# OpenNLPLab/ACR_WSSS

Measured on NVIDIA B200. Metric: train_imgs_per_sec, higher is better.
Workload: dtype bf16

## Files before the change

### acr_wsss_b200/csrc/attn_tc.cu

```cuda
#include "attn_tc.cuh"
#include <cstdlib>

using namespace acr_attn;

namespace {

struct FwdSmem {
  uint8_t q[TILE_BYTES];
  uint8_t k[2][TILE_BYTES];
  uint8_t v[2][TILE_BYTES];
  float mx[2][2][BM];
  float lsum[2][BM];
  uint64_t q_full, kv_full[2], kv_empty[2], s_full, s_free, p_full, o_full;
  uint32_t tmem_base;
};

constexpr float kRescaleThreshold = 8.f;
constexpr int FWD_THREADS = 384;
__device__ __forceinline__ void fwd_pair_sync(int quad) {
  switch (quad) {
    case 0: asm volatile("bar.sync 1, 64;" ::: "memory"); break;
    case 1: asm volatile("bar.sync 2, 64;" ::: "memory"); break;
    case 2: asm volatile("bar.sync 3, 64;" ::: "memory"); break;
    default: asm volatile("bar.sync 4, 64;" ::: "memory"); break;
  }
}
__global__ void __launch_bounds__(FWD_THREADS, 2)
attn_fwd_kernel(const __grid_constant__ CUtensorMap tmap_qkv, __nv_bfloat16* __restrict__ out, float* __restrict__ lse,
                int N, int H, float scale_log2) {
  extern __shared__ uint8_t smem_raw[];
  FwdSmem& s = *reinterpret_cast<FwdSmem*>((reinterpret_cast<uintptr_t>(smem_raw) + 1023) & ~(uintptr_t)1023);
  const int warp = threadIdx.x >> 5, lane = threadIdx.x & 31;
  const int q0 = blockIdx.x * BM, h = blockIdx.y, b = blockIdx.z;
  const int ntiles = (N + BN - 1) / BN;

  if (warp == 0 && lane == 0) {
    tc::prefetch_tmap(&tmap_qkv);
    tc::mbar_init(&s.q_full, 1);
    for (int i = 0; i < 2; ++i) { tc::mbar_init(&s.kv_full[i], 1); tc::mbar_init(&s.kv_empty[i], 1); }
    tc::mbar_init(&s.s_full, 1);
    tc::mbar_init(&s.s_free, 256);
    tc::mbar_init(&s.p_full, 256);
    tc::mbar_init(&s.o_full, 1);
    tc::fence_barrier_init();
  }
  if (warp == 2) tc::tmem_alloc<256>(&s.tmem_base);
  tc::tc_fence_before();
  __syncthreads();
  tc::tc_fence_after();
  const uint32_t tmem = s.tmem_base;
  const uint32_t tS = tmem, tP = tmem + 128, tO = tmem + 192;

  if (warp == 0) {
    tc::reg_dealloc<40>();
    if (tc::elect_one()) {
      tc::mbar_arrive_expect_tx(&s.q_full, TILE_BYTES);
      tc::tma_load_4d(s.q, &tmap_qkv, &s.q_full, 0, h, q0, b);
    }
    __syncwarp();
    for (int j = 0; j < ntiles; ++j) {
      const int st = j & 1;
      tc::mbar_wait(&s.kv_empty[st], ((j >> 1) & 1) ^ 1);
      if (tc::elect_one()) {
        tc::mbar_arrive_expect_tx(&s.kv_full[st], 2 * TILE_BYTES);
        tc::tma_load_4d(s.k[st], &tmap_qkv, &s.kv_full[st], 0, H + h, j * BN, b);
        tc::tma_load_4d(s.v[st], &tmap_qkv, &s.kv_full[st], 0, 2 * H + h, j * BN, b);
      }
      __syncwarp();
    }
  } else if (warp == 1) {
    tc::reg_dealloc<40>();
    tc::mbar_wait(&s.q_full, 0);
    const uint64_t qd = tc::smem_desc_sw128(tc::smem_u32(s.q), 16, 1024);
    auto issue_s = [&](int j) {
      const uint64_t kd = tc::smem_desc_sw128(tc::smem_u32(s.k[j & 1]), 16, 1024);
      if (tc::elect_one()) {
#pragma unroll
        for (int ks = 0; ks < HD / 16; ++ks) tc::mma_ss_off(tS, qd, ks * 2, kd, ks * 2, IDESC_S, ks > 0);
        tc::tc_commit(&s.s_full);
      }
      __syncwarp();
    };
    tc::mbar_wait(&s.kv_full[0], 0);
    tc::tc_fence_after();
    issue_s(0);
    for (int j = 0; j < ntiles; ++j) {
      const int st = j & 1;
      if (j + 1 < ntiles) {
        tc::mbar_wait(&s.kv_full[(j + 1) & 1], ((j + 1) >> 1) & 1);
        tc::mbar_wait(&s.s_free, j & 1);
        tc::tc_fence_after();
        issue_s(j + 1);
      }
      tc::mbar_wait(&s.p_full, j & 1);
      tc::tc_fence_after();
      const uint64_t vd = tc::smem_desc_sw128(tc::smem_u32(s.v[st]), 1024, 1024);
      if (tc::elect_one()) {
#pragma unroll
        for (int ks = 0; ks < BN / 16; ++ks) tc::mma_ts_off(tO, tP + ks * 8, vd, ks * 128, IDESC_PV, (j > 0) || (ks > 0));
        tc::tc_commit(&s.o_full);
        tc::tc_commit(&s.kv_empty[st]);
      }
      __syncwarp();
    }
  } else if (warp < 4) {
    tc::reg_dealloc<40>();
  } else {
    tc::reg_alloc<96>();
    const int half = (warp - 4) >> 2;
    const int quad = warp & 3;
    const int row = quad * 32 + lane;
    const uint32_t lane_off = (uint32_t)(quad * 32) << 16;
    const int cb = half * 64;
    float m = -INFINITY, l = 0.f;
    uint32_t r[32];
    const bool rows_live = q0 + quad * 32 < N;
    for (int j = 0; j < ntiles; ++j) {
      tc::mbar_wait(&s.s_full, j & 1);
      tc::tc_fence_after();
      if (!rows_live) {
        tc::tc_fence_before();
        tc::mbar_arrive(&s.s_free);
        tc::mbar_arrive(&s.p_full);
        tc::mbar_wait(&s.p_full, j & 1);
        continue;
      }
      const int ncols = min(BN, N - j * BN);
      const bool full = (ncols == BN);
      float mx = -INFINITY;
#pragma unroll
      for (int c = 0; c < 2; ++c) {
        const int c0 = cb + c * 32;
        if (c0 < ncols) {
          tc::tmem_ld32(tS + lane_off + c0, r);
          tc::tmem_ld_wait();
          if (full) {
#pragma unroll
            for (int i = 0; i < 32; ++i) mx = fmaxf(mx, __uint_as_float(r[i]));
          } else {
#pragma unroll
            for (int i = 0; i < 32; ++i) mx = fmaxf(mx, (c0 + i < ncols) ? __uint_as_float(r[i]) : -INFINITY);
          }
        }
      }
      s.mx[j & 1][half][row] = mx;
      fwd_pair_sync(quad);
      mx = fmaxf(mx, s.mx[j & 1][half ^ 1][row]);
      if (j > 0) {
        tc::mbar_wait(&s.o_full, (j - 1) & 1);
        tc::tc_fence_after();
      }
      if (j == 0) {
        m = mx;
      } else {
        const bool need = (mx - m) * scale_log2 > kRescaleThreshold;
        if (__any_sync(0xffffffffu, need)) {
          const float alpha = need ? tc::fast_exp2((m - mx) * scale_log2) : 1.f;
          if (need) { m = mx; l *= alpha; }
          tc::tmem_ld32(tO + lane_off + half * 32, r);
          tc::tmem_ld_wait();
#pragma unroll
          for (int i = 0; i < 32; ++i) r[i] = __float_as_uint(__uint_as_float(r[i]) * alpha);
          tc::tmem_st16(tO + lane_off + half * 32, r);
          tc::tmem_st16(tO + lane_off + half * 32 + 16, r + 16);
        }
      }
      const float ms = m * scale_log2;
      const uint64_t sc2 = tc::f2_pack(scale_log2, scale_log2), nms2 = tc::f2_pack(-ms, -ms);
      uint64_t rs2 = tc::f2_pack(0.f, 0.f);
#pragma unroll
      for (int c = 0; c < 2; ++c) {
        const int c0 = cb + c * 32;
        const bool any = c0 < ncols;
        if (any) {
          tc::tmem_ld32(tS + lane_off + c0, r);
          tc::tmem_ld_wait();
        }
        if (c == 1) {
          tc::tc_fence_before();
          tc::mbar_arrive(&s.s_free);
        }
        uint32_t pk[16];
        if (any) {
#pragma unroll
          for (int i = 0; i < 16; ++i) {
            float x0, x1;
            tc::f2_unpack(tc::f2_fma(tc::f2_pack(__uint_as_float(r[2 * i]), __uint_as_float(r[2 * i + 1])), sc2, nms2), x0, x1);
            float p0 = tc::fast_exp2(x0), p1 = tc::fast_exp2(x1);
            if (!full) {
              if (c0 + 2 * i >= ncols) p0 = 0.f;
              if (c0 + 2 * i + 1 >= ncols) p1 = 0.f;
            }
            rs2 = tc::f2_add(rs2, tc::f2_pack(p0, p1));
            pk[i] = tc::pack_bf16(p0, p1);
          }
        } else {
#pragma unroll
          for (int i = 0; i < 16; ++i) pk[i] = 0u;
        }
        tc::tmem_st16(tP + lane_off + half * 32 + c * 16, pk);
      }
      tc::tmem_st_wait();
      tc::tc_fence_before();
      tc::mbar_arrive(&s.p_full);
      float rs_lo, rs_hi;
      tc::f2_unpack(rs2, rs_lo, rs_hi);
      l += rs_lo + rs_hi;
    }
    if (rows_live) {
      s.lsum[half][row] = l;
      fwd_pair_sync(quad);
      l += s.lsum[half ^ 1][row];
      tc::mbar_wait(&s.o_full, (ntiles - 1) & 1);
      tc::tc_fence_after();
      tc::tmem_ld32(tO + lane_off + half * 32, r);
      tc::tmem_ld_wait();
      if (q0 + row < N) {
        const float inv = 1.f / l;
        __nv_bfloat16* dst = out + ((size_t)b * N + q0 + row) * ((size_t)H * HD) + (size_t)h * HD + half * 32;
#pragma unroll
        for (int c = 0; c < 4; ++c) {
          uint4 v;
          v.x = tc::pack_bf16(__uint_as_float(r[c * 8 + 0]) * inv, __uint_as_float(r[c * 8 + 1]) * inv);
          v.y = tc::pack_bf16(__uint_as_float(r[c * 8 + 2]) * inv, __uint_as_float(r[c * 8 + 3]) * inv);
          v.z = tc::pack_bf16(__uint_as_float(r[c * 8 + 4]) * inv, __uint_as_float(r[c * 8 + 5]) * inv);
          v.w = tc::pack_bf16(__uint_as_float(r[c * 8 + 6]) * inv, __uint_as_float(r[c * 8 + 7]) * inv);
          reinterpret_cast<uint4*>(dst)[c] = v;
        }
        if (half == 0) lse[((size_t)b * H + h) * N + q0 + row] = (m * scale_log2 + log2f(l)) * kLn2;
      }
    }
  }
  tc::tc_fence_before();
  __syncthreads();
  if (warp == 2) {
    tc::tc_fence_after();
    tc::tmem_dealloc<256>(tmem);
  }
}

constexpr int MEAN_STAGES = 3;
constexpr int MEAN_SW_SLICES = 4;
struct MeanSmem {
  uint8_t qk[MEAN_STAGES][2][TILE_BYTES];
  float lse2[MEAN_MAX_H][BM];
  float part[MEAN_SW_SLICES][MEAN_MAX_H][BM];
  uint64_t full[MEAN_STAGES], empty[MEAN_STAGES], t_full[2], t_empty[2];
  uint32_t tmem_base;
};
constexpr int STAGE_LD = 129;
static_assert(sizeof(float) * BM * STAGE_LD <= sizeof(uint8_t) * MEAN_STAGES * 2 * TILE_BYTES, "staging tile must fit");

constexpr int MEAN_SW = 16;
static_assert(MEAN_SW == 4 * MEAN_SW_SLICES, "slices of the softmax warps");
constexpr int MEAN_COLS = BN / (MEAN_SW / 4);
constexpr int MEAN_THREADS = 128 + MEAN_SW * 32;

template <int MODE>
__global__ void __launch_bounds__(MEAN_THREADS, 1)
attn_mean_kernel(const __grid_constant__ CUtensorMap tmap_qkv, const float* __restrict__ lse, float* __restrict__ mean,
                 long long mean_bs, long long mean_ld, GCode gc, float* __restrict__ p_row0, int N, int H, float scale_log2) {
  extern __shared__ uint8_t smem_raw[];
  MeanSmem& s = *reinterpret_cast<MeanSmem*>((reinterpret_cast<uintptr_t>(smem_raw) + 1023) & ~(uintptr_t)1023);
  const int warp = threadIdx.x >> 5, lane = threadIdx.x & 31;
  const int kv0 = blockIdx.x * BN, q0 = blockIdx.y * BM, b = blockIdx.z;

  if (warp == 0 && lane == 0) {
    tc::prefetch_tmap(&tmap_qkv);
    for (int i = 0; i < MEAN_STAGES; ++i) { tc::mbar_init(&s.full[i], 1); tc::mbar_init(&s.empty[i], 1); }
    for (int i = 0; i < 2; ++i) { tc::mbar_init(&s.t_full[i], 1); tc::mbar_init(&s.t_empty[i], MEAN_SW * 32); }
    tc::fence_barrier_init();
  }
  if (warp == 2) tc::tmem_alloc<256>(&s.tmem_base);
  tc::tc_fence_before();
  __syncthreads();
  tc::tc_fence_after();
  const uint32_t tmem = s.tmem_base;

  if (warp == 0) {
    for (int h = 0; h < H; ++h) {
      const int st = h % MEAN_STAGES;
      tc::mbar_wait(&s.empty[st], ((h / MEAN_STAGES) & 1) ^ 1);
      if (tc::elect_one()) {
        tc::mbar_arrive_expect_tx(&s.full[st], 2 * TILE_BYTES);
        tc::tma_load_4d(s.qk[st][0], &tmap_qkv, &s.full[st], 0, h, q0, b);
        tc::tma_load_4d(s.qk[st][1], &tmap_qkv, &s.full[st], 0, H + h, kv0, b);
      }
      __syncwarp();
    }
  } else if (warp == 1) {
    for (int h = 0; h < H; ++h) {
      const int st = h % MEAN_STAGES, ab = h & 1;
      tc::mbar_wait(&s.full[st], (h / MEAN_STAGES) & 1);
      tc::mbar_wait(&s.t_empty[ab], ((h >> 1) & 1) ^ 1);
      tc::tc_fence_after();
      const uint64_t qd = tc::smem_desc_sw128(tc::smem_u32(s.qk[st][0]), 16, 1024), kd = tc::smem_desc_sw128(tc::smem_u32(s.qk[st][1]), 16, 1024);
      if (tc::elect_one()) {
#pragma unroll
        for (int ks = 0; ks < HD / 16; ++ks) tc::mma_ss_off(tmem + ab * 128, qd, ks * 2, kd, ks * 2, IDESC_S, ks > 0);
        tc::tc_commit(&s.empty[st]);
        tc::tc_commit(&s.t_full[ab]);
      }
      __syncwarp();
    }
  } else if (warp >= 4) {
    const int we = warp - 4;
    const int row = (warp & 3) * 32 + lane;
    const int slice = we >> 2;
    const int sidx = we * 32 + lane;
    const uint32_t lane_off = (uint32_t)((warp & 3) * 32) << 16;
    const bool row_ok = (q0 + row) < N;
    const int col0 = kv0 + slice * MEAN_COLS;
    float acc[MEAN_COLS];
    const float invH = 1.f / (float)H;
    if (MODE == 0) {
#pragma unroll
      for (int i = 0; i < MEAN_COLS; ++i) acc[i] = 0.f;
    } else if (gc.ptr == nullptr) {
      const float* grow = mean + (size_t)b * mean_bs + (size_t)(q0 + row) * mean_ld + col0;
#pragma unroll
      for (int i = 0; i < MEAN_COLS; ++i) acc[i] = (row_ok && col0 + i < N) ? __ldg(grow + i) * invH : 0.f;
    } else {
      const float w2 = gcode_weight(gc, q0 + row, invH);
      const uint4* crow = reinterpret_cast<const uint4*>(gc.ptr + (size_t)b * gc.bs + (size_t)min(q0 + row, N - 1) * gc.ld + col0);
#pragma unroll
      for (int v = 0; v < MEAN_COLS / 16; ++v) {
        const uint4 t = __ldg(crow + v);
        const uint32_t w[4] = {t.x, t.y, t.z, t.w};
#pragma unroll
        for (int j = 0; j < 4; ++j)
#pragma unroll
          for (int k = 0; k < 4; ++k) {
            const int i = v * 16 + j * 4 + k;
            acc[i] = (row_ok && col0 + i < N) ? ACR_CODE_F(w[j], k) * w2 : 0.f;
          }
      }
    }
    {
      constexpr int HSTEP = MEAN_SW * 32 / BM;
      const int rr = sidx & (BM - 1);
      const bool ok = (q0 + rr) < N;
      const float* lp = lse + (size_t)b * H * N + q0 + rr;
      for (int h0 = sidx / BM; h0 < H; h0 += HSTEP * 4) {
        float v[4];
#pragma unroll
        for (int k = 0; k < 4; ++k) v[k] = (ok && h0 + HSTEP * k < H) ? __ldg(lp + (size_t)(h0 + HSTEP * k) * N) : INFINITY;
#pragma unroll
        for (int k = 0; k < 4; ++k)
          if (h0 + HSTEP * k < H) s.lse2[h0 + HSTEP * k][rr] = v[k] * kLog2e;
      }
    }
    asm volatile("bar.sync 1, %0;" ::"n"(MEAN_SW * 32) : "memory");
    const bool tail = (kv0 + BN > N);
    const bool row0_warp = (MODE == 0) && (p_row0 != nullptr) && (q0 == 0) && ((warp & 3) == 0);
    const bool live = (q0 + (warp & 3) * 32 < N) && (col0 < N);
    uint32_t r[32];
    for (int h = 0; h < H; ++h) {
      const int ab = h & 1;
      const float lse2 = s.lse2[h][row];
      tc::mbar_wait(&s.t_full[ab], (h >> 1) & 1);
      tc::tc_fence_after();
      float part = 0.f;
#pragma unroll
      for (int c = 0; c < MEAN_COLS / 32; ++c) {
        const int colbase = col0 + c * 32;
        if (!live || (tail && colbase >= N)) break;
        tc::tmem_ld32(tmem + ab * 128 + lane_off + slice * MEAN_COLS + c * 32, r);
        tc::tmem_ld_wait();
        if (!tail) {
          const uint64_t sc2 = tc::f2_pack(scale_log2, scale_log2), nl2 = tc::f2_pack(-lse2, -lse2);
          uint64_t part2 = tc::f2_pack(0.f, 0.f);
#pragma unroll
          for (int i = 0; i < 32; i += 2) {
            float x0, x1;
            tc::f2_unpack(tc::f2_fma(tc::f2_pack(__uint_as_float(r[i]), __uint_as_float(r[i + 1])), sc2, nl2), x0, x1);
            const float p0 = tc::fast_exp2(x0), p1 = tc::fast_exp2(x1);
            const uint64_t pp = tc::f2_pack(p0, p1), aa = tc::f2_pack(acc[c * 32 + i], acc[c * 32 + i + 1]);
            if (MODE == 0) {
              tc::f2_unpack(tc::f2_add(aa, pp), acc[c * 32 + i], acc[c * 32 + i + 1]);
              r[i] = __float_as_uint(p0); r[i + 1] = __float_as_uint(p1);
            } else {
              part2 = tc::f2_fma(pp, aa, part2);
            }
          }
          if (MODE == 1) { float a0, a1; tc::f2_unpack(part2, a0, a1); part += a0 + a1; }
        } else {
#pragma unroll
          for (int i = 0; i < 32; ++i) {
            float p = tc::fast_exp2(fmaf(__uint_as_float(r[i]), scale_log2, -lse2));
            if (colbase + i >= N) p = 0.f;
            if (MODE == 0) { acc[c * 32 + i] += p; r[i] = __float_as_uint(p); } else part = fmaf(p, acc[c * 32 + i], part);
          }
        }
        if (row0_warp && lane == 0) {
          float* dst0 = p_row0 + ((size_t)b * H + h) * N + colbase;
#pragma unroll
          for (int i = 0; i < 32; ++i)
            if (colbase + i < N) dst0[i] = __uint_as_float(r[i]);
        }
      }
      tc::tc_fence_before();
      tc::mbar_arrive(&s.t_empty[ab]);
      if (MODE == 1) s.part[slice][h][row] = part;
    }
    if (MODE == 1) {
      asm volatile("bar.sync 1, %0;" ::"n"(MEAN_SW * 32) : "memory");
      float* plane = p_row0 + (size_t)blockIdx.x * gridDim.z * H * N;
      for (int idx = sidx; idx < H * BM; idx += MEAN_SW * 32) {
        const int hh = idx / BM, rr = idx % BM;
        if (q0 + rr < N) {
          float v = 0.f;
#pragma unroll
          for (int sl = 0; sl < MEAN_SW_SLICES; ++sl) v += s.part[sl][hh][rr];
          plane[((size_t)b * H + hh) * N + q0 + rr] = v;
        }
      }
    }
    if (MODE == 0) {
    float* stage = reinterpret_cast<float*>(&s.qk[0][0][0]);
#pragma unroll
    for (int i = 0; i < MEAN_COLS; ++i) stage[row * STAGE_LD + slice * MEAN_COLS + i] = acc[i] * invH;
    asm volatile("bar.sync 1, %0;" ::"n"(MEAN_SW * 32) : "memory");
    float* dst = mean + (size_t)b * mean_bs;
    constexpr int RPW = BM / MEAN_SW;
#pragma unroll 1
    for (int r4 = we * RPW; r4 < we * RPW + RPW; r4 += 4) {
      if (q0 + r4 >= N) break;
      float v[4][4];
#pragma unroll
      for (int u = 0; u < 4; ++u)
#pragma unroll
        for (int cc = 0; cc < 4; ++cc) v[u][cc] = stage[(r4 + u) * STAGE_LD + cc * 32 + lane];
#pragma unroll
      for (int u = 0; u < 4; ++u) {
        if (q0 + r4 + u < N) {
#pragma unroll
          for (int cc = 0; cc < 4; ++cc) {
            const int col = cc * 32 + lane;
            if (kv0 + col < N) dst[(size_t)(q0 + r4 + u) * N + kv0 + col] = v[u][cc];
          }
        }
      }
    }
    }
  }
  tc::tc_fence_before();
  __syncthreads();
  if (warp == 2) {
    tc::tc_fence_after();
    tc::tmem_dealloc<256>(tmem);
  }
}

}

namespace acr_attn {
EncodeTiledFn get_encode_fn() {
  static EncodeTiledFn fn = nullptr;
  if (!fn) {
    void* p = nullptr;
    cudaDriverEntryPointQueryResult qres;
    if (cudaGetDriverEntryPoint("cuTensorMapEncodeTiled", &p, cudaEnableDefault, &qres) != cudaSuccess || qres != cudaDriverEntryPointSuccess)
      return nullptr;
    fn = (EncodeTiledFn)p;
  }
  return fn;
}

int make_tmap(CUtensorMap* m, const void* base, int B, int N, int SH, int D) {
  EncodeTiledFn fn = get_encode_fn();
  ACR_REQUIRE(fn != nullptr, ACR_E_NOSM100, "cuTensorMapEncodeTiled unavailable");
  cuuint64_t dims[4] = {(cuuint64_t)D, (cuuint64_t)SH, (cuuint64_t)N, (cuuint64_t)B};
  cuuint64_t strides[3] = {(cuuint64_t)D * 2, (cuuint64_t)SH * D * 2, (cuuint64_t)N * SH * D * 2};
  cuuint32_t box[4] = {(cuuint32_t)D, 1, (cuuint32_t)BM, 1};
  cuuint32_t estr[4] = {1, 1, 1, 1};
  CUresult r = fn(m, CU_TENSOR_MAP_DATA_TYPE_BFLOAT16, 4, const_cast<void*>(base), dims, strides, box, estr, CU_TENSOR_MAP_INTERLEAVE_NONE,
                  CU_TENSOR_MAP_SWIZZLE_128B, CU_TENSOR_MAP_L2_PROMOTION_L2_256B, CU_TENSOR_MAP_FLOAT_OOB_FILL_NONE);
  ACR_REQUIRE(r == CUDA_SUCCESS, ACR_E_INVAL, "cuTensorMapEncodeTiled failed (%d)", (int)r);
  return 0;
}

}

extern "C" int acr_attn_fwd_bf16(const void* qkv, int B, int N, int H, int D, float scale,
                                 void* out, float* lse, float* attn_mean, long long mean_batch_stride,
                                 float* p_row0, void* stream) {
  ACR_REQUIRE(qkv && out && lse, ACR_E_INVAL, "acr_attn_fwd_bf16: null pointer");
  ACR_REQUIRE(B > 0 && N > 0 && H > 0, ACR_E_INVAL, "acr_attn_fwd_bf16: bad shape");
  ACR_REQUIRE(D == HD, ACR_E_INVAL, "acr_attn_fwd_bf16: head dim %d unsupported (64 only)", D);
  ACR_REQUIRE(B <= 65535 && H <= MEAN_MAX_H, ACR_E_INVAL, "acr_attn_fwd_bf16: B <= 65535 and H <= %d required", MEAN_MAX_H);
  ACR_REQUIRE(((uintptr_t)qkv & 15) == 0 && ((uintptr_t)out & 15) == 0, ACR_E_ALIGN, "acr_attn_fwd_bf16: qkv/out must be 16-byte aligned");
  ACR_REQUIRE(p_row0 == nullptr || attn_mean != nullptr, ACR_E_INVAL, "acr_attn_fwd_bf16: p_row0 needs attn_mean");
  ACR_REQUIRE(acr_device_is_sm100(), ACR_E_NOSM100, "acr_attn_fwd_bf16: needs an sm_100 device");
  cudaStream_t st = (cudaStream_t)stream;
  CUtensorMap tmap;
  if (int e = make_tmap(&tmap, qkv, B, N, 3 * H, D)) return e;
  const float scale_log2 = scale * kLog2e;
  const int qt = (N + BM - 1) / BM, kt = (N + BN - 1) / BN;
  {
    const size_t smem = sizeof(FwdSmem) + 1024;
    static bool attr_set[64] = {false};
    if (int e = set_max_smem(attn_fwd_kernel, smem, attr_set)) return e;
    dim3 grid(qt, H, B);
    acr::KernelTimer kt_("attn_fwd_kernel", st);
    attn_fwd_kernel<<<grid, FWD_THREADS, smem, st>>>(tmap, (__nv_bfloat16*)out, lse, N, H, scale_log2);
    if (int e = acr::check_launch("attn_fwd_kernel")) return e;
  }
  if (attn_mean) {
    const size_t smem = sizeof(MeanSmem) + 1024;
    static bool attr_set[64] = {false};
    if (int e = set_max_smem(attn_mean_kernel<0>, smem, attr_set)) return e;
    dim3 grid(kt, qt, B);
    acr::KernelTimer kt_("attn_mean_kernel", st);
    attn_mean_kernel<0><<<grid, MEAN_THREADS, smem, st>>>(tmap, lse, attn_mean, mean_batch_stride, (long long)N, GCode{}, p_row0, N, H, scale_log2);
    if (int e = acr::check_launch("attn_mean_kernel")) return e;
  }
  return 0;
}


namespace {


__global__ void __launch_bounds__(256)
bwd_delta_kernel(const __nv_bfloat16* __restrict__ out, const __nv_bfloat16* __restrict__ d_out, const float* __restrict__ part,
                 int nparts, float* __restrict__ delta, float4* __restrict__ dq_acc, int* __restrict__ dq_bad, long long rows, int N, int H) {
  const int lane = threadIdx.x & 31;
  const long long t = ((long long)blockIdx.x * (blockDim.x >> 5) + (threadIdx.x >> 5)) * 4 + (lane >> 3);
  const bool ok = t < rows;
  float acc = 0.f;
  if (ok) {
    const uint4 a = __ldg(reinterpret_cast<const uint4*>(out + t * HD) + (lane & 7));
    const uint4 d = __ldg(reinterpret_cast<const uint4*>(d_out + t * HD) + (lane & 7));
    const __nv_bfloat162* a2 = reinterpret_cast<const __nv_bfloat162*>(&a);
    const __nv_bfloat162* d2 = reinterpret_cast<const __nv_bfloat162*>(&d);
#pragma unroll
    for (int i = 0; i < 4; ++i) {
      const float2 fa = __bfloat1622float2(a2[i]), fd = __bfloat1622float2(d2[i]);
      acc = fmaf(fa.x, fd.x, acc);
      acc = fmaf(fa.y, fd.y, acc);
    }
    const float4 z = make_float4(0.f, 0.f, 0.f, 0.f);
#pragma unroll
    for (int m = 0; m < 4; ++m) dq_acc[t * (HD / 2) + m * 8 + (lane & 7)] = z;
  }
  acc += __shfl_xor_sync(0xffffffffu, acc, 1);
  acc += __shfl_xor_sync(0xffffffffu, acc, 2);
  acc += __shfl_xor_sync(0xffffffffu, acc, 4);
  if (ok && (lane & 7) == 0) {
    const int h = (int)(t % H);
    const long long bn = t / H;
    const int n = (int)(bn % N), b = (int)(bn / N);
    const size_t idx = ((size_t)b * H + h) * N + n;
    for (int k = 0; k < nparts; ++k) acc += __ldg(part + (size_t)k * rows + idx);
    delta[idx] = acc;
    dq_bad[idx] = 0;
  }
}

__global__ void __launch_bounds__(256)
bwd_dq_convert_kernel(const long long* __restrict__ dq_acc, const int* __restrict__ dq_bad, __nv_bfloat16* __restrict__ d_qkv, int B, int N,
                      int H, float scale) {
  const long long t = (long long)blockIdx.x * blockDim.x + threadIdx.x;
  if (t >= (long long)B * H * N * (HD / 8)) return;
  const int c = (int)(t % (HD / 8));
  const long long row = t / (HD / 8);
  const int n = (int)(row % N);
  const int h = (int)((row / N) % H);
  const int b = (int)(row / ((long long)N * H));
  const longlong2* src = reinterpret_cast<const longlong2*>(dq_acc + row * HD + c * 8);
  const float sc = __ldg(dq_bad + row) ? __int_as_float(0x7fc00000) : scale * kDqUnfix;
  float x[8];
#pragma unroll
  for (int j = 0; j < 4; ++j) {
    const longlong2 q = __ldg(src + j);
    x[2 * j] = __ll2float_rn(q.x) * sc;
    x[2 * j + 1] = __ll2float_rn(q.y) * sc;
  }
  uint4 v;
  v.x = tc::pack_bf16(x[0], x[1]);
  v.y = tc::pack_bf16(x[2], x[3]);
  v.z = tc::pack_bf16(x[4], x[5]);
  v.w = tc::pack_bf16(x[6], x[7]);
  *reinterpret_cast<uint4*>(d_qkv + (((size_t)b * N + n) * 3 + 0) * ((size_t)H * HD) + (size_t)h * HD + c * 8) = v;
}

}

extern "C" size_t acr_attn_bwd_bf16_workspace(int B, int N, int H, int D) {
  if (B <= 0 || N <= 0 || H <= 0 || D <= 0) return 0;
  const size_t rows = (size_t)B * H * N, kt = (N + BN - 1) / BN;
  return acr::align_up(rows * sizeof(float), 256) + acr::align_up(rows * D * sizeof(long long), 256) + acr::align_up(kt * rows * sizeof(float), 256) +
         acr::align_up(rows * sizeof(int), 256);
}

extern "C" int acr_attn_bwd_bf16(const void* qkv, const void* out, const float* lse, const void* d_out,
                                 int B, int N, int H, int D, float scale,
                                 const float* g_mean, long long g_batch_stride, long long g_row_stride,
                                 const unsigned char* g_code, long long code_batch_stride, long long code_row_stride,
                                 float w_cls, float w_aff, const float* g_scale,
                                 void* d_qkv, float* g_row0, void* workspace, size_t workspace_bytes, void* stream) {
  ACR_REQUIRE(qkv && out && lse && d_out && d_qkv && workspace, ACR_E_INVAL, "acr_attn_bwd_bf16: null pointer");
  ACR_REQUIRE(B > 0 && N > 0 && H > 0, ACR_E_INVAL, "acr_attn_bwd_bf16: bad shape");
  ACR_REQUIRE(D == HD, ACR_E_INVAL, "acr_attn_bwd_bf16: head dim %d unsupported (64 only)", D);
  ACR_REQUIRE(B <= 65535 && H <= MEAN_MAX_H, ACR_E_INVAL, "acr_attn_bwd_bf16: B <= 65535 and H <= %d required", MEAN_MAX_H);
  ACR_REQUIRE(g_mean == nullptr || g_row_stride >= N, ACR_E_INVAL, "acr_attn_bwd_bf16: g_row_stride < N");
  ACR_REQUIRE(g_mean == nullptr || g_code == nullptr, ACR_E_INVAL, "acr_attn_bwd_bf16: give g_mean OR g_code");
  ACR_REQUIRE(g_code == nullptr || ((code_row_stride % 128) == 0 && code_row_stride >= (long long)((N + 127) / 128) * 128 &&
                                    (code_batch_stride % 16) == 0 && ((uintptr_t)g_code & 15) == 0),
              ACR_E_ALIGN, "acr_attn_bwd_bf16: g_code rows must be 128-byte padded and 16-byte aligned");
  const GCode gc{g_code, code_batch_stride, code_row_stride, w_cls, w_aff, g_scale};
  ACR_REQUIRE(((uintptr_t)qkv & 15) == 0 && ((uintptr_t)out & 15) == 0 && ((uintptr_t)d_out & 15) == 0 && ((uintptr_t)d_qkv & 15) == 0,
              ACR_E_ALIGN, "acr_attn_bwd_bf16: tensors must be 16-byte aligned");
  ACR_REQUIRE(((uintptr_t)workspace & 255) == 0, ACR_E_ALIGN, "acr_attn_bwd_bf16: workspace must be 256-byte aligned");
  ACR_REQUIRE(workspace_bytes >= acr_attn_bwd_bf16_workspace(B, N, H, D), ACR_E_NOMEM, "acr_attn_bwd_bf16: workspace too small");
  ACR_REQUIRE(acr_device_is_sm100(), ACR_E_NOSM100, "acr_attn_bwd_bf16: needs an sm_100 device");
  cudaStream_t st = (cudaStream_t)stream;
  const size_t rows = (size_t)B * H * N;
  const int qt = (N + BM - 1) / BM, kt = (N + BN - 1) / BN;
  float* delta = (float*)workspace;
  long long* dq_acc = (long long*)((char*)workspace + acr::align_up(rows * sizeof(float), 256));
  float* delta_part = (float*)((char*)dq_acc + acr::align_up(rows * D * sizeof(long long), 256));
  int* dq_bad = (int*)((char*)delta_part + acr::align_up((size_t)kt * rows * sizeof(float), 256));
  CUtensorMap tmap_qkv, tmap_do, tmap_dq;
  if (int e = make_tmap(&tmap_qkv, qkv, B, N, 3 * H, D)) return e;
  if (int e = make_tmap(&tmap_do, d_out, B, N, H, D)) return e;
  {
    EncodeTiledFn fn = get_encode_fn();
    ACR_REQUIRE(fn != nullptr, ACR_E_NOSM100, "cuTensorMapEncodeTiled unavailable");
    cuuint64_t dims[3] = {(cuuint64_t)HD, (cuuint64_t)N, (cuuint64_t)B * H};
    cuuint64_t strides[2] = {(cuuint64_t)HD * 8, (cuuint64_t)N * HD * 8};
    cuuint32_t box[3] = {16, (cuuint32_t)BM, 1};
    cuuint32_t estr[3] = {1, 1, 1};
    CUresult r = fn(&tmap_dq, CU_TENSOR_MAP_DATA_TYPE_UINT64, 3, dq_acc, dims, strides, box, estr, CU_TENSOR_MAP_INTERLEAVE_NONE,
                    CU_TENSOR_MAP_SWIZZLE_128B, CU_TENSOR_MAP_L2_PROMOTION_NONE, CU_TENSOR_MAP_FLOAT_OOB_FILL_NONE);
    ACR_REQUIRE(r == CUDA_SUCCESS, ACR_E_INVAL, "cuTensorMapEncodeTiled(dq) failed (%d)", (int)r);
  }
  const float scale_log2 = scale * kLog2e;

  const bool with_g = g_mean || g_code;
  if (with_g) {
    const size_t smem = sizeof(MeanSmem) + 1024;
    static bool attr_set[64] = {false};
    if (int e = set_max_smem(attn_mean_kernel<1>, smem, attr_set)) return e;
    dim3 grid(kt, qt, B);
    acr::KernelTimer kt_("attn_delta_kernel", st);
    attn_mean_kernel<1><<<grid, MEAN_THREADS, smem, st>>>(tmap_qkv, lse, const_cast<float*>(g_mean), g_batch_stride, g_row_stride, gc, delta_part, N, H, scale_log2);
    if (int e = acr::check_launch("attn_mean_kernel<1>")) return e;
  }
  bwd_delta_kernel<<<(unsigned)((rows + 31) / 32), 256, 0, st>>>((const __nv_bfloat16*)out, (const __nv_bfloat16*)d_out, delta_part,
                                                               with_g ? kt : 0, delta, reinterpret_cast<float4*>(dq_acc), dq_bad, (long long)rows, N, H);
  if (int e = acr::check_launch("bwd_delta_kernel")) return e;
  if (int e = launch_attn_bwd(tmap_qkv, tmap_do, tmap_dq, lse, delta, g_mean, g_batch_stride, g_row_stride, gc, (__nv_bfloat16*)d_qkv, g_row0, dq_bad, B, N, H, scale, st))
    return e;
  const long long nconv = (long long)rows * (HD / 8);
  bwd_dq_convert_kernel<<<(unsigned)((nconv + 255) / 256), 256, 0, st>>>(dq_acc, dq_bad, (__nv_bfloat16*)d_qkv, B, N, H, scale);
  return acr::check_launch("bwd_dq_convert_kernel");
}
```

### acr_wsss_b200/csrc/attn_tc.cuh

```cuda
#pragma once
#include "common.cuh"
#include "tc_common.cuh"

namespace acr_attn {

constexpr int BM = 128;
constexpr int BN = 128;
constexpr int HD = 64;
constexpr uint32_t TILE_BYTES = BM * HD * 2;
constexpr float kLog2e = 1.4426950408889634f;
constexpr float kLn2 = 0.6931471805599453f;
constexpr int MEAN_MAX_H = 32;
constexpr float kDqFix = 1099511627776.0f;
constexpr float kDqUnfix = 1.0f / 1099511627776.0f;
inline float dq_fix_limit(int kt) {
  int lg = 0;
  while ((1 << lg) < kt) ++lg;
  return ldexpf(1.0f, 62 - lg);
}

constexpr uint32_t IDESC_S = tc::idesc_bf16_f32(128, 128, 0, 0);
constexpr uint32_t IDESC_PV = tc::idesc_bf16_f32(128, 64, 0, 1);
constexpr uint32_t IDESC_DQ = tc::idesc_bf16_f32(128, 64, 1, 1);

struct GCode {
  const unsigned char* ptr;
  long long bs, ld;
  float w_cls, w_aff;
  const float* scale;
};
__device__ __forceinline__ float gcode_weight(const GCode& gc, int q, float invH) {
  const float sc = gc.scale ? __ldg(gc.scale) : 1.f;
  return 2.f * invH * sc * (q == 0 ? gc.w_cls : gc.w_aff);
}
#define ACR_CODE_F(word, k) __uint_as_float(__byte_perm((word), 0u, 0x0444u | ((k) << 12)))

typedef CUresult (*EncodeTiledFn)(CUtensorMap*, CUtensorMapDataType, cuuint32_t, void*, const cuuint64_t*, const cuuint64_t*,
                                  const cuuint32_t*, const cuuint32_t*, CUtensorMapInterleave, CUtensorMapSwizzle,
                                  CUtensorMapL2promotion, CUtensorMapFloatOOBfill);
EncodeTiledFn get_encode_fn();
int make_tmap(CUtensorMap* m, const void* base, int B, int N, int SH, int D);

template <typename K>
int set_max_smem(K kernel, size_t bytes, bool* done ) {
  int dev = 0;
  ACR_CUDA(cudaGetDevice(&dev));
  if (dev >= 0 && dev < 64 && done[dev]) return 0;
  ACR_CUDA(cudaFuncSetAttribute(kernel, cudaFuncAttributeMaxDynamicSharedMemorySize, (int)bytes));
  if (dev >= 0 && dev < 64) done[dev] = true;
  return 0;
}

int launch_attn_bwd(const CUtensorMap& tmap_qkv, const CUtensorMap& tmap_do, const CUtensorMap& tmap_dq, const float* lse, const float* delta,
                    const float* g_mean, long long g_bs, long long g_ld, const GCode& gc, __nv_bfloat16* d_qkv, float* g_row0,
                    int* dq_bad, int B, int N, int H, float scale, cudaStream_t st);

}
```

Measured before the change: 590.2.

## Shrink head-mean kernel to 64-column tiles with two CTAs per SM

Restructures the head-mean/delta kernel to use 64-wide KV tiles with 8 softmax warps instead of 128-wide tiles with 16. Shared memory is now sized dynamically by H, and register budgets are rebalanced with reg_dealloc/reg_alloc, so that two CTAs fit per SM. A producer-side warp preloads the LSE values. The delta partial buffer layout is changed to three planes per 128-tile, so the bwd_delta reduction keeps its per-128-tile indexing, and the workspace grows to match. The aim is higher occupancy and better latency hiding. The cost is more CTAs, more duplicated Q loads, and a more complex partial-sum layout.

```diff
diff --git a/acr_wsss_b200/csrc/attn_tc.cu b/acr_wsss_b200/csrc/attn_tc.cu
--- a/acr_wsss_b200/csrc/attn_tc.cu
+++ b/acr_wsss_b200/csrc/attn_tc.cu
@@ -239,76 +239,110 @@
   }
 }
 
+constexpr int MEAN_BN = 64;
 constexpr int MEAN_STAGES = 3;
-constexpr int MEAN_SW_SLICES = 4;
+constexpr uint32_t MEAN_K_BYTES = MEAN_BN * HD * 2;
+constexpr int MEAN_SLICES = 2;
+constexpr int MEAN_COLS = MEAN_BN / MEAN_SLICES;
+constexpr int MEAN_SW = 4 * MEAN_SLICES;
+constexpr int MEAN_THREADS = 128 + MEAN_SW * 32;
+constexpr uint32_t IDESC_S64 = tc::idesc_bf16_f32(128, MEAN_BN, 0, 0);
 struct MeanSmem {
-  uint8_t qk[MEAN_STAGES][2][TILE_BYTES];
-  float lse2[MEAN_MAX_H][BM];
-  float part[MEAN_SW_SLICES][MEAN_MAX_H][BM];
+  uint8_t q[MEAN_STAGES][TILE_BYTES];
+  uint8_t k[MEAN_STAGES][MEAN_K_BYTES];
   uint64_t full[MEAN_STAGES], empty[MEAN_STAGES], t_full[2], t_empty[2];
   uint32_t tmem_base;
 };
-constexpr int STAGE_LD = 129;
-static_assert(sizeof(float) * BM * STAGE_LD <= sizeof(uint8_t) * MEAN_STAGES * 2 * TILE_BYTES, "staging tile must fit");
-
-constexpr int MEAN_SW = 16;
-static_assert(MEAN_SW == 4 * MEAN_SW_SLICES, "slices of the softmax warps");
-constexpr int MEAN_COLS = BN / (MEAN_SW / 4);
-constexpr int MEAN_THREADS = 128 + MEAN_SW * 32;
+constexpr int STAGE_LD = MEAN_BN + 1;
+static_assert(sizeof(float) * BM * STAGE_LD <= sizeof(MeanSmem::q), "staging tile must fit");
+constexpr size_t mean_smem_bytes(int mode, int H) {
+  return sizeof(MeanSmem) + sizeof(float) * BM * H * (mode == 1 ? 1 + MEAN_SLICES : 1) + 1024;
+}
+static_assert(2 * (mean_smem_bytes(1, 16) + 1024) <= 228 * 1024 && 2 * (mean_smem_bytes(0, 16) + 1024) <= 228 * 1024,
+              "two head-mean / delta CTAs must fit one SM at H <= 16 (ViT-B, ViT-L)");
 
 template <int MODE>
-__global__ void __launch_bounds__(MEAN_THREADS, 1)
-attn_mean_kernel(const __grid_constant__ CUtensorMap tmap_qkv, const float* __restrict__ lse, float* __restrict__ mean,
-                 long long mean_bs, long long mean_ld, GCode gc, float* __restrict__ p_row0, int N, int H, float scale_log2) {
+__global__ void __launch_bounds__(MEAN_THREADS, 2)
+attn_mean_kernel(const __grid_constant__ CUtensorMap tmap_q, const __grid_constant__ CUtensorMap tmap_k, const float* __restrict__ lse,
+                 float* __restrict__ mean, long long mean_bs, long long mean_ld, GCode gc, float* __restrict__ p_row0, int N, int H,
+                 float scale_log2) {
   extern __shared__ uint8_t smem_raw[];
   MeanSmem& s = *reinterpret_cast<MeanSmem*>((reinterpret_cast<uintptr_t>(smem_raw) + 1023) & ~(uintptr_t)1023);
+  float* lse2s = reinterpret_cast<float*>(&s + 1);
+  float* parts = lse2s + H * BM;
   const int warp = threadIdx.x >> 5, lane = threadIdx.x & 31;
-  const int kv0 = blockIdx.x * BN, q0 = blockIdx.y * BM, b = blockIdx.z;
+  const int kv0 = blockIdx.x * MEAN_BN, q0 = blockIdx.y * BM, b = blockIdx.z;
 
   if (warp == 0 && lane == 0) {
-    tc::prefetch_tmap(&tmap_qkv);
+    tc::prefetch_tmap(&tmap_q);
+    tc::prefetch_tmap(&tmap_k);
     for (int i = 0; i < MEAN_STAGES; ++i) { tc::mbar_init(&s.full[i], 1); tc::mbar_init(&s.empty[i], 1); }
     for (int i = 0; i < 2; ++i) { tc::mbar_init(&s.t_full[i], 1); tc::mbar_init(&s.t_empty[i], MEAN_SW * 32); }
     tc::fence_barrier_init();
   }
-  if (warp == 2) tc::tmem_alloc<256>(&s.tmem_base);
+  if (warp == 2) tc::tmem_alloc<2 * MEAN_BN>(&s.tmem_base);
   tc::tc_fence_before();
   __syncthreads();
   tc::tc_fence_after();
   const uint32_t tmem = s.tmem_base;
 
-  if (warp == 0) {
-    for (int h = 0; h < H; ++h) {
-      const int st = h % MEAN_STAGES;
-      tc::mbar_wait(&s.empty[st], ((h / MEAN_STAGES) & 1) ^ 1);
-      if (tc::elect_one()) {
-        tc::mbar_arrive_expect_tx(&s.full[st], 2 * TILE_BYTES);
-        tc::tma_load_4d(s.qk[st][0], &tmap_qkv, &s.full[st], 0, h, q0, b);
-        tc::tma_load_4d(s.qk[st][1], &tmap_qkv, &s.full[st], 0, H + h, kv0, b);
-      }
-      __syncwarp();
-    }
-  } else if (warp == 1) {
-    for (int h = 0; h < H; ++h) {
-      const int st = h % MEAN_STAGES, ab = h & 1;
-      tc::mbar_wait(&s.full[st], (h / MEAN_STAGES) & 1);
-      tc::mbar_wait(&s.t_empty[ab], ((h >> 1) & 1) ^ 1);
-      tc::tc_fence_after();
-      const uint64_t qd = tc::smem_desc_sw128(tc::smem_u32(s.qk[st][0]), 16, 1024), kd = tc::smem_desc_sw128(tc::smem_u32(s.qk[st][1]), 16, 1024);
-      if (tc::elect_one()) {
-#pragma unroll
-        for (int ks = 0; ks < HD / 16; ++ks) tc::mma_ss_off(tmem + ab * 128, qd, ks * 2, kd, ks * 2, IDESC_S, ks > 0);
-        tc::tc_commit(&s.empty[st]);
-        tc::tc_commit(&s.t_full[ab]);
-      }
-      __syncwarp();
-    }
-  } else if (warp >= 4) {
+  if (warp < 4) {
+    tc::reg_dealloc<40>();
+    if (warp == 0) {
+      for (int h = 0; h < H; ++h) {
+        const int st = h % MEAN_STAGES;
+        tc::mbar_wait(&s.empty[st], ((h / MEAN_STAGES) & 1) ^ 1);
+        if (tc::elect_one()) {
+          tc::mbar_arrive_expect_tx(&s.full[st], TILE_BYTES + MEAN_K_BYTES);
+          tc::tma_load_4d(s.q[st], &tmap_q, &s.full[st], 0, h, q0, b);
+          tc::tma_load_4d(s.k[st], &tmap_k, &s.full[st], 0, H + h, kv0, b);
+        }
+        __syncwarp();
+      }
+    } else if (warp == 1) {
+      for (int h = 0; h < H; ++h) {
+        const int st = h % MEAN_STAGES, ab = h & 1;
+        tc::mbar_wait(&s.full[st], (h / MEAN_STAGES) & 1);
+        tc::mbar_wait(&s.t_empty[ab], ((h >> 1) & 1) ^ 1);
+        tc::tc_fence_after();
+        const uint64_t qd = tc::smem_desc_sw128(tc::smem_u32(s.q[st]), 16, 1024), kd = tc::smem_desc_sw128(tc::smem_u32(s.k[st]), 16, 1024);
+        if (tc::elect_one()) {
+#pragma unroll
+          for (int ks = 0; ks < HD / 16; ++ks) tc::mma_ss_off(tmem + ab * MEAN_BN, qd, ks * 2, kd, ks * 2, IDESC_S64, ks > 0);
+          tc::tc_commit(&s.empty[st]);
+          tc::tc_commit(&s.t_full[ab]);
+        }
+        __syncwarp();
+      }
+    } else {
+      const int rr = threadIdx.x - 64;
+      const bool ok0 = q0 + rr < N, ok1 = q0 + rr + 64 < N;
+      const float* lp = lse + (size_t)b * H * N + q0 + rr;
+      for (int h0 = 0; h0 < H; h0 += 4) {
+        float v[4][2];
+#pragma unroll
+        for (int k = 0; k < 4; ++k) {
+          const bool hk = h0 + k < H;
+          v[k][0] = (hk && ok0) ? __ldg(lp + (size_t)(h0 + k) * N) : INFINITY;
+          v[k][1] = (hk && ok1) ? __ldg(lp + (size_t)(h0 + k) * N + 64) : INFINITY;
+        }
+#pragma unroll
+        for (int k = 0; k < 4; ++k)
+          if (h0 + k < H) {
+            lse2s[(h0 + k) * BM + rr] = v[k][0] * kLog2e;
+            lse2s[(h0 + k) * BM + rr + 64] = v[k][1] * kLog2e;
+          }
+      }
+      asm volatile("bar.sync 1, %0;" ::"n"(MEAN_THREADS - 64) : "memory");
+    }
+  } else {
+    tc::reg_alloc<96>();
     const int we = warp - 4;
-    const int row = (warp & 3) * 32 + lane;
+    const int quad = warp & 3;
+    const int row = quad * 32 + lane;
     const int slice = we >> 2;
     const int sidx = we * 32 + lane;
-    const uint32_t lane_off = (uint32_t)((warp & 3) * 32) << 16;
+    const uint32_t lane_off = (uint32_t)(quad * 32) << 16;
     const bool row_ok = (q0 + row) < N;
     const int col0 = kv0 + slice * MEAN_COLS;
     float acc[MEAN_COLS];
@@ -336,36 +370,20 @@
           }
       }
     }
-    {
-      constexpr int HSTEP = MEAN_SW * 32 / BM;
-      const int rr = sidx & (BM - 1);
-      const bool ok = (q0 + rr) < N;
-      const float* lp = lse + (size_t)b * H * N + q0 + rr;
-      for (int h0 = sidx / BM; h0 < H; h0 += HSTEP * 4) {
-        float v[4];
-#pragma unroll
-        for (int k = 0; k < 4; ++k) v[k] = (ok && h0 + HSTEP * k < H) ? __ldg(lp + (size_t)(h0 + HSTEP * k) * N) : INFINITY;
-#pragma unroll
-        for (int k = 0; k < 4; ++k)
-          if (h0 + HSTEP * k < H) s.lse2[h0 + HSTEP * k][rr] = v[k] * kLog2e;
-      }
-    }
-    asm volatile("bar.sync 1, %0;" ::"n"(MEAN_SW * 32) : "memory");
-    const bool tail = (kv0 + BN > N);
-    const bool row0_warp = (MODE == 0) && (p_row0 != nullptr) && (q0 == 0) && ((warp & 3) == 0);
-    const bool live = (q0 + (warp & 3) * 32 < N) && (col0 < N);
+    asm volatile("bar.sync 1, %0;" ::"n"(MEAN_THREADS - 64) : "memory");
+    const bool tail = (kv0 & ~(BN - 1)) + BN > N;
+    const bool row0_warp = (MODE == 0) && (p_row0 != nullptr) && (q0 == 0) && (quad == 0);
+    const bool live = (q0 + quad * 32 < N) && (col0 < N);
+    const uint32_t tcol = lane_off + slice * MEAN_COLS;
     uint32_t r[32];
     for (int h = 0; h < H; ++h) {
       const int ab = h & 1;
-      const float lse2 = s.lse2[h][row];
+      const float lse2 = lse2s[h * BM + row];
       tc::mbar_wait(&s.t_full[ab], (h >> 1) & 1);
       tc::tc_fence_after();
       float part = 0.f;
-#pragma unroll
-      for (int c = 0; c < MEAN_COLS / 32; ++c) {
-        const int colbase = col0 + c * 32;
-        if (!live || (tail && colbase >= N)) break;
-        tc::tmem_ld32(tmem + ab * 128 + lane_off + slice * MEAN_COLS + c * 32, r);
+      if (live) {
+        tc::tmem_ld32(tmem + ab * MEAN_BN + tcol, r);
         tc::tmem_ld_wait();
         if (!tail) {
           const uint64_t sc2 = tc::f2_pack(scale_log2, scale_log2), nl2 = tc::f2_pack(-lse2, -lse2);
@@ -375,9 +393,9 @@
             float x0, x1;
             tc::f2_unpack(tc::f2_fma(tc::f2_pack(__uint_as_float(r[i]), __uint_as_float(r[i + 1])), sc2, nl2), x0, x1);
             const float p0 = tc::fast_exp2(x0), p1 = tc::fast_exp2(x1);
-            const uint64_t pp = tc::f2_pack(p0, p1), aa = tc::f2_pack(acc[c * 32 + i], acc[c * 32 + i + 1]);
+            const uint64_t pp = tc::f2_pack(p0, p1), aa = tc::f2_pack(acc[i], acc[i + 1]);
             if (MODE == 0) {
-              tc::f2_unpack(tc::f2_add(aa, pp), acc[c * 32 + i], acc[c * 32 + i + 1]);
+              tc::f2_unpack(tc::f2_add(aa, pp), acc[i], acc[i + 1]);
               r[i] = __float_as_uint(p0); r[i + 1] = __float_as_uint(p1);
             } else {
               part2 = tc::f2_fma(pp, aa, part2);
@@ -388,67 +406,73 @@
 #pragma unroll
           for (int i = 0; i < 32; ++i) {
             float p = tc::fast_exp2(fmaf(__uint_as_float(r[i]), scale_log2, -lse2));
-            if (colbase + i >= N) p = 0.f;
-            if (MODE == 0) { acc[c * 32 + i] += p; r[i] = __float_as_uint(p); } else part = fmaf(p, acc[c * 32 + i], part);
+            if (col0 + i >= N) p = 0.f;
+            if (MODE == 0) { acc[i] += p; r[i] = __float_as_uint(p); } else part = fmaf(p, acc[i], part);
           }
         }
         if (row0_warp && lane == 0) {
-          float* dst0 = p_row0 + ((size_t)b * H + h) * N + colbase;
+          float* dst0 = p_row0 + ((size_t)b * H + h) * N + col0;
 #pragma unroll
           for (int i = 0; i < 32; ++i)
-            if (colbase + i < N) dst0[i] = __uint_as_float(r[i]);
+            if (col0 + i < N) dst0[i] = __uint_as_float(r[i]);
         }
       }
       tc::tc_fence_before();
       tc::mbar_arrive(&s.t_empty[ab]);
-      if (MODE == 1) s.part[slice][h][row] = part;
+      if (MODE == 1) parts[(slice * H + h) * BM + row] = part;
     }
     if (MODE == 1) {
-      asm volatile("bar.sync 1, %0;" ::"n"(MEAN_SW * 32) : "memory");
-      float* plane = p_row0 + (size_t)blockIdx.x * gridDim.z * H * N;
+      asm volatile("bar.sync 2, %0;" ::"n"(MEAN_SW * 32) : "memory");
+      const size_t pstride = (size_t)gridDim.z * H * N;
+      const bool odd = blockIdx.x & 1;
+      float* plane = p_row0 + (size_t)(3 * (blockIdx.x >> 1) + odd) * pstride;
       for (int idx = sidx; idx < H * BM; idx += MEAN_SW * 32) {
         const int hh = idx / BM, rr = idx % BM;
         if (q0 + rr < N) {
-          float v = 0.f;
-#pragma unroll
-          for (int sl = 0; sl < MEAN_SW_SLICES; ++sl) v += s.part[sl][hh][rr];
-          plane[((size_t)b * H + hh) * N + q0 + rr] = v;
+          const float s0 = parts[hh * BM + rr], s1 = parts[(H + hh) * BM + rr];
+          const size_t o = ((size_t)b * H + hh) * N + q0 + rr;
+          if (odd) {
+            plane[o] = s0;
+            plane[o + pstride] = s1;
+          } else {
+            plane[o] = (0.f + s0) + s1;
+          }
         }
       }
     }
     if (MODE == 0) {
-    float* stage = reinterpret_cast<float*>(&s.qk[0][0][0]);
-#pragma unroll
-    for (int i = 0; i < MEAN_COLS; ++i) stage[row * STAGE_LD + slice * MEAN_COLS + i] = acc[i] * invH;
-    asm volatile("bar.sync 1, %0;" ::"n"(MEAN_SW * 32) : "memory");
-    float* dst = mean + (size_t)b * mean_bs;
-    constexpr int RPW = BM / MEAN_SW;
+      float* stage = reinterpret_cast<float*>(&s.q[0][0]);
+#pragma unroll
+      for (int i = 0; i < MEAN_COLS; ++i) stage[row * STAGE_LD + slice * MEAN_COLS + i] = acc[i] * invH;
+      asm volatile("bar.sync 2, %0;" ::"n"(MEAN_SW * 32) : "memory");
+      float* dst = mean + (size_t)b * mean_bs;
+      constexpr int RPW = BM / MEAN_SW;
 #pragma unroll 1
-    for (int r4 = we * RPW; r4 < we * RPW + RPW; r4 += 4) {
-      if (q0 + r4 >= N) break;
-      float v[4][4];
-#pragma unroll
-      for (int u = 0; u < 4; ++u)
-#pragma unroll
-        for (int cc = 0; cc < 4; ++cc) v[u][cc] = stage[(r4 + u) * STAGE_LD + cc * 32 + lane];
-#pragma unroll
-      for (int u = 0; u < 4; ++u) {
-        if (q0 + r4 + u < N) {
-#pragma unroll
-          for (int cc = 0; cc < 4; ++cc) {
-            const int col = cc * 32 + lane;
-            if (kv0 + col < N) dst[(size_t)(q0 + r4 + u) * N + kv0 + col] = v[u][cc];
-          }
-        }
-      }
-    }
+      for (int r4 = we * RPW; r4 < we * RPW + RPW; r4 += 4) {
+        if (q0 + r4 >= N) break;
+        float v[4][MEAN_SLICES];
+#pragma unroll
+        for (int u = 0; u < 4; ++u)
+#pragma unroll
+          for (int cc = 0; cc < MEAN_SLICES; ++cc) v[u][cc] = stage[(r4 + u) * STAGE_LD + cc * 32 + lane];
+#pragma unroll
+        for (int u = 0; u < 4; ++u) {
+          if (q0 + r4 + u < N) {
+#pragma unroll
+            for (int cc = 0; cc < MEAN_SLICES; ++cc) {
+              const int col = cc * 32 + lane;
+              if (kv0 + col < N) dst[(size_t)(q0 + r4 + u) * N + kv0 + col] = v[u][cc];
+            }
+          }
+        }
+      }
     }
   }
   tc::tc_fence_before();
   __syncthreads();
   if (warp == 2) {
     tc::tc_fence_after();
-    tc::tmem_dealloc<256>(tmem);
+    tc::tmem_dealloc<2 * MEAN_BN>(tmem);
   }
 }
 
@@ -467,12 +491,12 @@
   return fn;
 }
 
-int make_tmap(CUtensorMap* m, const void* base, int B, int N, int SH, int D) {
+int make_tmap(CUtensorMap* m, const void* base, int B, int N, int SH, int D, int box_rows) {
   EncodeTiledFn fn = get_encode_fn();
   ACR_REQUIRE(fn != nullptr, ACR_E_NOSM100, "cuTensorMapEncodeTiled unavailable");
   cuuint64_t dims[4] = {(cuuint64_t)D, (cuuint64_t)SH, (cuuint64_t)N, (cuuint64_t)B};
   cuuint64_t strides[3] = {(cuuint64_t)D * 2, (cuuint64_t)SH * D * 2, (cuuint64_t)N * SH * D * 2};
-  cuuint32_t box[4] = {(cuuint32_t)D, 1, (cuuint32_t)BM, 1};
+  cuuint32_t box[4] = {(cuuint32_t)D, 1, (cuuint32_t)box_rows, 1};
   cuuint32_t estr[4] = {1, 1, 1, 1};
   CUresult r = fn(m, CU_TENSOR_MAP_DATA_TYPE_BFLOAT16, 4, const_cast<void*>(base), dims, strides, box, estr, CU_TENSOR_MAP_INTERLEAVE_NONE,
                   CU_TENSOR_MAP_SWIZZLE_128B, CU_TENSOR_MAP_L2_PROMOTION_L2_256B, CU_TENSOR_MAP_FLOAT_OOB_FILL_NONE);
@@ -496,7 +520,7 @@
   CUtensorMap tmap;
   if (int e = make_tmap(&tmap, qkv, B, N, 3 * H, D)) return e;
   const float scale_log2 = scale * kLog2e;
-  const int qt = (N + BM - 1) / BM, kt = (N + BN - 1) / BN;
+  const int qt = (N + BM - 1) / BM;
   {
     const size_t smem = sizeof(FwdSmem) + 1024;
     static bool attr_set[64] = {false};
@@ -507,12 +531,14 @@
     if (int e = acr::check_launch("attn_fwd_kernel")) return e;
   }
   if (attn_mean) {
-    const size_t smem = sizeof(MeanSmem) + 1024;
+    CUtensorMap tmap_k;
+    if (int e = make_tmap(&tmap_k, qkv, B, N, 3 * H, D, MEAN_BN)) return e;
     static bool attr_set[64] = {false};
-    if (int e = set_max_smem(attn_mean_kernel<0>, smem, attr_set)) return e;
-    dim3 grid(kt, qt, B);
+    if (int e = set_max_smem(attn_mean_kernel<0>, mean_smem_bytes(0, MEAN_MAX_H), attr_set)) return e;
+    dim3 grid((N + MEAN_BN - 1) / MEAN_BN, qt, B);
     acr::KernelTimer kt_("attn_mean_kernel", st);
-    attn_mean_kernel<0><<<grid, MEAN_THREADS, smem, st>>>(tmap, lse, attn_mean, mean_batch_stride, (long long)N, GCode{}, p_row0, N, H, scale_log2);
+    attn_mean_kernel<0><<<grid, MEAN_THREADS, mean_smem_bytes(0, H), st>>>(tmap, tmap_k, lse, attn_mean, mean_batch_stride, (long long)N, GCode{},
+                                                                          p_row0, N, H, scale_log2);
     if (int e = acr::check_launch("attn_mean_kernel")) return e;
   }
   return 0;
@@ -524,7 +550,7 @@
 
 __global__ void __launch_bounds__(256)
 bwd_delta_kernel(const __nv_bfloat16* __restrict__ out, const __nv_bfloat16* __restrict__ d_out, const float* __restrict__ part,
-                 int nparts, float* __restrict__ delta, float4* __restrict__ dq_acc, int* __restrict__ dq_bad, long long rows, int N, int H) {
+                 int ntiles, float* __restrict__ delta, float4* __restrict__ dq_acc, int* __restrict__ dq_bad, long long rows, int N, int H) {
   const int lane = threadIdx.x & 31;
   const long long t = ((long long)blockIdx.x * (blockDim.x >> 5) + (threadIdx.x >> 5)) * 4 + (lane >> 3);
   const bool ok = t < rows;
@@ -552,7 +578,15 @@
     const long long bn = t / H;
     const int n = (int)(bn % N), b = (int)(bn / N);
     const size_t idx = ((size_t)b * H + h) * N + n;
-    for (int k = 0; k < nparts; ++k) acc += __ldg(part + (size_t)k * rows + idx);
+    const int nhalf = (N + 63) / 64;
+    for (int k = 0; k < ntiles; ++k) {
+      const float* pk = part + (size_t)3 * k * rows + idx;
+      const bool odd = 2 * k + 1 < nhalf;
+      float v = __ldg(pk);
+      v += odd ? __ldg(pk + rows) : 0.f;
+      v += odd ? __ldg(pk + 2 * rows) : 0.f;
+      acc += v;
+    }
     delta[idx] = acc;
     dq_bad[idx] = 0;
   }
@@ -590,7 +624,7 @@
 extern "C" size_t acr_attn_bwd_bf16_workspace(int B, int N, int H, int D) {
   if (B <= 0 || N <= 0 || H <= 0 || D <= 0) return 0;
   const size_t rows = (size_t)B * H * N, kt = (N + BN - 1) / BN;
-  return acr::align_up(rows * sizeof(float), 256) + acr::align_up(rows * D * sizeof(long long), 256) + acr::align_up(kt * rows * sizeof(float), 256) +
+  return acr::align_up(rows * sizeof(float), 256) + acr::align_up(rows * D * sizeof(long long), 256) + acr::align_up(3 * kt * rows * sizeof(float), 256) +
          acr::align_up(rows * sizeof(int), 256);
 }
 
@@ -621,7 +655,7 @@
   float* delta = (float*)workspace;
   long long* dq_acc = (long long*)((char*)workspace + acr::align_up(rows * sizeof(float), 256));
   float* delta_part = (float*)((char*)dq_acc + acr::align_up(rows * D * sizeof(long long), 256));
-  int* dq_bad = (int*)((char*)delta_part + acr::align_up((size_t)kt * rows * sizeof(float), 256));
+  int* dq_bad = (int*)((char*)delta_part + acr::align_up((size_t)3 * kt * rows * sizeof(float), 256));
   CUtensorMap tmap_qkv, tmap_do, tmap_dq;
   if (int e = make_tmap(&tmap_qkv, qkv, B, N, 3 * H, D)) return e;
   if (int e = make_tmap(&tmap_do, d_out, B, N, H, D)) return e;
@@ -640,12 +674,14 @@
 
   const bool with_g = g_mean || g_code;
   if (with_g) {
-    const size_t smem = sizeof(MeanSmem) + 1024;
+    CUtensorMap tmap_k;
+    if (int e = make_tmap(&tmap_k, qkv, B, N, 3 * H, D, MEAN_BN)) return e;
     static bool attr_set[64] = {false};
-    if (int e = set_max_smem(attn_mean_kernel<1>, smem, attr_set)) return e;
-    dim3 grid(kt, qt, B);
+    if (int e = set_max_smem(attn_mean_kernel<1>, mean_smem_bytes(1, MEAN_MAX_H), attr_set)) return e;
+    dim3 grid((N + MEAN_BN - 1) / MEAN_BN, qt, B);
     acr::KernelTimer kt_("attn_delta_kernel", st);
-    attn_mean_kernel<1><<<grid, MEAN_THREADS, smem, st>>>(tmap_qkv, lse, const_cast<float*>(g_mean), g_batch_stride, g_row_stride, gc, delta_part, N, H, scale_log2);
+    attn_mean_kernel<1><<<grid, MEAN_THREADS, mean_smem_bytes(1, H), st>>>(tmap_qkv, tmap_k, lse, const_cast<float*>(g_mean), g_batch_stride,
+                                                                          g_row_stride, gc, delta_part, N, H, scale_log2);
     if (int e = acr::check_launch("attn_mean_kernel<1>")) return e;
   }
   bwd_delta_kernel<<<(unsigned)((rows + 31) / 32), 256, 0, st>>>((const __nv_bfloat16*)out, (const __nv_bfloat16*)d_out, delta_part,
diff --git a/acr_wsss_b200/csrc/attn_tc.cuh b/acr_wsss_b200/csrc/attn_tc.cuh
--- a/acr_wsss_b200/csrc/attn_tc.cuh
+++ b/acr_wsss_b200/csrc/attn_tc.cuh
@@ -39,7 +39,7 @@
                                   const cuuint32_t*, const cuuint32_t*, CUtensorMapInterleave, CUtensorMapSwizzle,
                                   CUtensorMapL2promotion, CUtensorMapFloatOOBfill);
 EncodeTiledFn get_encode_fn();
-int make_tmap(CUtensorMap* m, const void* base, int B, int N, int SH, int D);
+int make_tmap(CUtensorMap* m, const void* base, int B, int N, int SH, int D, int box_rows = BM);
 
 template <typename K>
 int set_max_smem(K kernel, size_t bytes, bool* done ) {
```

Result: no change. 590.4, median of 6 (+0.0%).
